# DataIntensive-HPC/abft-sparse-cg

Measured on AMD Instinct MI355X. Metric: CG iterations/sec + SpMV effective HBM GB/s (% of roofline), 1/2/4/8 MI355X, higher is better.
Workload: dtype f64; 1 GPU; cg-csr -t hip -m none, synthetic laplace5:3162,3162; N=9998244, nnz=49978572, format=csr, mode=none, parallelism=1 GPU

## Files before the change

### abft_sparse_cg_amd/capi.py

```python
import ctypes as C
import os

_HERE = os.path.dirname(os.path.abspath(__file__))
LIB_PATH = os.environ.get("ABFT_HIP_LIB") or os.path.join(_HERE, "libabft_hip.so")
HEADER_PATH = os.path.join(os.path.dirname(_HERE), "include", "abft_hip.h")

OK = 0
MODES = ("none", "constraints", "sed", "sec7", "sec8", "secded")
MODE_ID = {m: i for i, m in enumerate(MODES)}
MODE_ID["sec"] = MODE_ID["sec7"]
FMT_CSR, FMT_COO = 0, 1
FLIP_ANY, FLIP_VALUE, FLIP_INDEX = 0, 1, 2
PART_ALL, PART_INTERIOR, PART_BOUNDARY = 0, 1, 2
K_SPMV, K_DOT, K_CALC_XR, K_CALC_P = 0, 1, 2, 3
EV_VEC_CORRECTED, EV_VEC_DOUBLE = 10, 11
FMT_VECTOR = 2
MAX_RHS = 8

u32p = C.POINTER(C.c_uint32)
f64p = C.POINTER(C.c_double)
i32p = C.POINTER(C.c_int)
vp = C.c_void_p
vpp = C.POINTER(C.c_void_p)

# ... 78 lines not shown
    "abft_hip_calc_px_precond_block": (C.c_int, [vp, vp, vp, vp, vp, C.c_int, f64p, f64p, C.c_uint32]),
    "abft_hip_dot_dev": (C.c_int, [vp, vp, vp, vp]),
    "abft_hip_calc_xr_dev": (C.c_int, [vp, vp, vp, vp, vp, C.c_double, vp]),
    "abft_hip_read_pair": (C.c_int, [vp, vp, f64p, f64p]),
    "abft_hip_spmv_dot_dev": (C.c_int, [vp, vp, vp, vp, C.c_int, vp]),
    "abft_hip_matrix_set_interior": (C.c_int, [vp, C.c_int, C.c_int]),
    "abft_hip_spmv_part": (C.c_int, [vp, vp, vp, vp, C.c_int]),
    "abft_hip_spmv_dot_part_dev": (C.c_int, [vp, vp, vp, vp, C.c_int, vp, C.c_int]),
    "abft_hip_calc_xr_ratio_dev": (C.c_int, [vp, vp, vp, vp, vp, vp, vp, vp]),
    "abft_hip_calc_p_ratio_dev": (C.c_int, [vp, vp, vp, vp, vp]),
    "abft_hip_set_sharers": (C.c_int, [vp, C.c_int]),
    "abft_hip_speculation_stats": (C.c_int, [vp, C.POINTER(C.c_long), C.POINTER(C.c_long)]),
    "abft_hip_cg_iteration_dev": (C.c_int, [vp, vp, vp, C.c_int, C.c_int, vp, vp, vp, vp, vp, vp, vp]),
    "abft_hip_tail_stats": (C.c_int, [vp, i32p, i32p, i32p, C.POINTER(C.c_long)]),
    "abft_hip_x_in_spmv_stats": (C.c_int, [vp, C.POINTER(C.c_long), C.POINTER(C.c_long)]),
    "abft_hip_cg_iteration_until_dev": (C.c_int, [vp, vp, vp, C.c_int, C.c_int, vp, vp, vp, vp, vp, vp, vp, C.c_double]),
    "abft_hip_write_pair": (C.c_int, [vp, vp, C.c_double, C.c_double]),
    "abft_hip_peer_board_bytes": (C.c_size_t, []),
    "abft_hip_peer_board_attach": (C.c_int, [vp, vp, C.c_size_t, C.c_int, C.c_int, C.c_double]),
    "abft_hip_peer_board_detach": (C.c_int, [vp]),
    "abft_hip_allreduce_pair_peers": (C.c_int, [vp, vp]),
    "abft_hip_peer_board_failed": (C.c_int, [vp]),
    "abft_hip_peer_board_ipc_handle_bytes": (C.c_size_t, []),
    "abft_hip_peer_board_ipc_export": (C.c_int, [vp, vp]),
    "abft_hip_peer_board_ipc_attach": (C.c_int, [vp, vp, C.c_int, C.c_int, C.c_double]),
    "abft_hip_peer_board_device_alloc": (C.c_int, [vp, C.POINTER(vp)]),
    "abft_hip_peer_board_device_free": (C.c_int, [vp, vp]),
    "abft_hip_peer_board_attach_device": (C.c_int, [vp, C.POINTER(vp), C.c_int, C.c_int, C.c_double]),
    "abft_hip_peer_board_fuse": (C.c_int, [vp, C.c_int]),
    "abft_hip_peer_exchange_bytes": (C.c_size_t, [C.c_int, C.c_size_t]),
# ... 81 lines not shown
```

### abft_sparse_cg_amd/context.py

```python
import ctypes as C
import math
import sys

import numpy as np

from . import capi
from .capi import FMT_COO, FMT_CSR, MODE_ID, check


class FatalEvent(SystemExit):

    def __init__(self, events):
        super().__init__(1)
        self.events = events


class ResidualCheckFailed(RuntimeError):

    def __init__(self, message, checks):
        super().__init__(message)
        self.checks = checks


class Matrix:
# ... 424 lines not shown
    def stream_probe(self, nbytes=1 << 30, reps=10):
        c, r = C.c_double(), C.c_double()
        check(self.L.abft_hip_stream_probe(self.h, nbytes, reps, C.byref(c), C.byref(r)))
        return c.value, r.value

    def tail_stats(self):
        path, grid, want = C.c_int(0), C.c_int(0), C.c_int(0)
        counts = (C.c_long * 4)()
        check(self.L.abft_hip_tail_stats(self.h, C.byref(path), C.byref(grid), C.byref(want), counts))
        return path.value, grid.value, want.value, list(counts)

    def x_in_spmv_stats(self):
        absorbed, flushed = C.c_long(0), C.c_long(0)
        check(self.L.abft_hip_x_in_spmv_stats(self.h, C.byref(absorbed), C.byref(flushed)))
        return absorbed.value, flushed.value

    def cg_iteration_until_dev(self, mat, vec, x, r, p, w, scalars, rr_at, pw_at, rr_new_at, threshold, vec_offset=0,
                               part=capi.PART_ALL):
        base = scalars.device_ptr
        check(self.L.abft_hip_cg_iteration_until_dev(self.h, mat.h, vec.h, vec_offset, part, x.h, r.h, p.h, w.h,
                                                     base + 8 * rr_at, base + 8 * pw_at, base + 8 * rr_new_at,
                                                     threshold))

    def graph_begin(self):
        check(self.L.abft_hip_graph_begin(self.h))

    def graph_end(self):
        g = C.c_void_p()
        check(self.L.abft_hip_graph_end(self.h, C.byref(g)))
        return g
# ... 368 lines not shown
```

### abft_sparse_cg_amd/csrc/abft_hip.hip

```cpp
#include <algorithm>
#include <array>
#include <chrono>
#include <cmath>
#include <cstdarg>
#include <cstdio>
#include <cstdlib>
#include <cstring>
#include <new>
#include <thread>
#include <map>
#include <mutex>
#include <vector>

#include "abft_internal.h"


static thread_local char g_err[512] = "";

static int set_err(int code, const char *fmt, ...) {
  va_list ap;
  va_start(ap, fmt);
  vsnprintf(g_err, sizeof(g_err), fmt, ap);
  va_end(ap);
  return code;
// ... 36 lines not shown
  HostSlot *host_slot_dev = nullptr;
  struct {
    bool enabled = false;
    bool learned = false;
    abft_hip_vector *x = nullptr, *r = nullptr, *p = nullptr, *w = nullptr;
    bool have_rr = false;
    int rr_at = 0;
    double rr_host = 0.0;
    int stage = 0;
    uint32_t seq_rr = 0;
    double rr_new_host = 0.0;
    double *shadow[2] = {nullptr, nullptr};
    int shadow_n = 0;
    double *scal = nullptr;
    long commits = 0, drops = 0;
  } spec;
  EventRing ring{};
  MovedList moved{};
  int *bits_dev = nullptr;
  bool fuse_enabled = true;
  struct {
    bool valid = false, have_value = false;
    bool vecc = false;
    const double *x = nullptr, *y = nullptr;
    int n = 0;
    uint32_t seq = 0;
    double value = 0.0;
  } fused;
  bool defer_enabled = true;
  struct {
// ... 115 lines not shown
  return ABFT_OK;
}

static int flush_deferred(abft_hip_ctx *ctx) {
  if (!ctx->defer.active) return ABFT_OK;
  ctx->defer.active = false;
  HIPCHK(launch_axpy(ctx->defer.x, ctx->defer.p, ctx->defer.alpha, ctx->defer.on_dev ? ctx->alpha_dev : nullptr,
                     ctx->defer.n, ctx->stream));
  return ABFT_OK;
}

static bool same_bits(double a, double b) { return memcmp(&a, &b, sizeof(a)) == 0; }

static void spec_drop(abft_hip_ctx *ctx) {
  auto &S = ctx->spec;
  if (S.stage) S.drops++;
  if (S.stage == 2) {
    S.rr_at = 1 - S.rr_at;
    S.rr_host = S.rr_new_host;
  }
  S.stage = 0;
}
static void spec_forget(abft_hip_ctx *ctx) {
  spec_drop(ctx);
  ctx->spec.learned = false;
  ctx->spec.have_rr = false;
  ctx->spec.x = ctx->spec.r = ctx->spec.p = ctx->spec.w = nullptr;
}

static int bind(abft_hip_ctx *ctx, bool keep_deferred = false, bool keep_spec = false, bool keep_xpend = false) {
  if (!ctx) return set_err(ABFT_ERR_INVALID, "null context");
  HIPCHK(hipSetDevice(ctx->device));
  ctx->xpend.prev_p = ctx->xpend.last_p;
  ctx->xpend.last_p = nullptr;
  if (!keep_spec) spec_drop(ctx);
  if (!keep_deferred && !keep_xpend)
    if (int rc = flush_xpend(ctx)) return rc;
  if (!keep_deferred) return flush_deferred(ctx);
  return ABFT_OK;
}
// ... 120 lines not shown
  if (const char *e = getenv("ABFT_HIP_TAIL")) ctx->tail_enabled = strcmp(e, "0") != 0;
  if (const char *e = getenv("ABFT_HIP_SYNC")) ctx->spin_wait = strcmp(e, "stream") != 0;
  if (const char *e = getenv("ABFT_HIP_FUSE_DOT")) ctx->fuse_enabled = strcmp(e, "0") != 0;
  if (const char *e = getenv("ABFT_HIP_FUSE_X")) ctx->defer_enabled = strcmp(e, "0") != 0;
  HIPCHK(hipMalloc((void **)&ctx->alpha_dev, sizeof(double)));
  HIPCHK(hipHostMalloc((void **)&ctx->host_slot, ABFT_HOST_SLOTS * sizeof(HostSlot), hipHostMallocMapped | hipHostMallocCoherent));
  memset(ctx->host_slot, 0, ABFT_HOST_SLOTS * sizeof(HostSlot));
  HIPCHK(hipMalloc((void **)&ctx->spec.scal, 8 * sizeof(double)));
  HIPCHK(hipMemset(ctx->spec.scal, 0, 8 * sizeof(double)));
  if (const char *e = getenv("ABFT_HIP_SPECULATE")) ctx->spec.enabled = strcmp(e, "0") != 0;
  if (const char *e = getenv("ABFT_HIP_X_IN_SPMV")) {
    ctx->xin_enabled = strcmp(e, "0") != 0;
    if (ctx->xin_enabled) ctx->xin_modes = ~0u;
  }
  ctx->xin_enabled = ctx->xin_enabled && ctx->defer_enabled && ctx->fuse_enabled && !ctx->spec.enabled;
  HIPCHK(hipHostGetDevicePointer((void **)&ctx->host_slot_dev, ctx->host_slot, 0));
  HIPCHK(hipMalloc((void **)&ctx->ring.buf, EVENT_CAP * sizeof(abft_event) + VECC_SEEN_BYTES));
  HIPCHK(hipMalloc((void **)&ctx->ring.count, sizeof(uint32_t)));
  HIPCHK(hipMemset(ctx->ring.count, 0, sizeof(uint32_t)));
  HIPCHK(hipMemset(ctx->ring.buf + EVENT_CAP, 0, VECC_SEEN_BYTES));
  ctx->ring.cap = EVENT_CAP;
  HIPCHK(hipMalloc((void **)&ctx->moved.buf, 2 * (size_t)MOVED_CAP * sizeof(MovedEntry)));
  HIPCHK(hipMalloc((void **)&ctx->moved.count, sizeof(uint32_t)));
  HIPCHK(hipMemset(ctx->moved.count, 0, sizeof(uint32_t)));
  ctx->moved.cap = MOVED_CAP;
  HIPCHK(hipMalloc((void **)&ctx->bits_dev, 32 * sizeof(int)));
  {
    double *scratch = nullptr;
    HIPCHK(hipMalloc((void **)&scratch, 8 * sizeof(double)));
    HIPCHK(hipMemset(scratch, 0, 8 * sizeof(double)));
// ... 1414 lines not shown
                     disjoint(x, p) && disjoint(x, w) && disjoint(r, p);
  KernelTimer t(ctx, ABFT_K_CALC_XR);
  if (defer) {
    HIPCHK(launch_calc_r(r->d, w->d, alpha, num, den, num ? ctx->alpha_dev : nullptr, x->n, o, ctx->stream, nullptr, x->d, p->d));
    ctx->defer.active = true;
    ctx->defer.on_dev = num != nullptr;
    ctx->defer.x = x->d; ctx->defer.p = p->d; ctx->defer.n = x->n; ctx->defer.alpha = alpha;
    return ABFT_OK;
  }
  HIPCHK(launch_calc_xr(x->d, r->d, p->d, w->d, alpha, num, den, x->n, o, ctx->stream));
  return ABFT_OK;
}

static bool spec_plain(const abft_hip_vector *v, int n);

static bool xpend_take(abft_hip_ctx *ctx, abft_hip_vector *p, const abft_hip_vector *r, double beta, int *rc) {
  auto &X = ctx->xpend;
  *rc = ABFT_OK;
  if (!ctx->xin_enabled || !X.armed || X.active || ctx->defer.on_dev || ctx->capturing) return false;
  if (!spec_plain(p, p->n) || !disjoint(p, r)) return false;
  int at = X.shadow[0].buf && X.shadow[0].n == p->n ? 0 : X.shadow[1].buf && X.shadow[1].n == p->n ? 1 : -1;
  if (at < 0) {
    at = X.shadow[X.shadow_at].buf ? 1 - X.shadow_at : X.shadow_at;
    (void)hipFree(X.shadow[at].buf);
    X.shadow[at].buf = nullptr;
    X.shadow[at].n = 0;
    if (hipMalloc((void **)&X.shadow[at].buf, ((size_t)p->n + 2) * sizeof(double)) != hipSuccess) {
      (void)hipGetLastError();
      X.shadow[at].buf = nullptr;
      ctx->xin_enabled = false;
      return false;
    }
    X.shadow[at].n = p->n;
  }
  X.shadow_at = at;
  {
    KernelTimer t(ctx, ABFT_K_CALC_P);
    const hipError_t e = launch_calc_p(p->d, r->d, beta, nullptr, nullptr, p->n, ctx->stream, X.shadow[at].buf);
    if (e != hipSuccess) {
      *rc = set_err(ABFT_ERR_HIP, "calc_p: %s", hipGetErrorString(e));
      return true;
    }
  }
  std::swap(p->d, X.shadow[at].buf);
  X.active = true;
  X.x = ctx->defer.x; X.p_old = X.shadow[at].buf; X.alpha = ctx->defer.alpha; X.n = p->n; X.ph = p;
  return true;
}

static int calc_p_launch(abft_hip_ctx *ctx, abft_hip_vector *p, const abft_hip_vector *r, double beta,
// ... 13 lines not shown
        ctx->xpend.last_p = p;
        if (taken) return ABFT_OK;
      }
      KernelTimer t(ctx, ABFT_K_CALC_P);
      HIPCHK(launch_calc_px(p->d, r->d, ctx->defer.x, beta, num, den, ctx->defer.alpha,
                            ctx->defer.on_dev ? ctx->alpha_dev : nullptr, p->n, ctx->stream));
      return ABFT_OK;
    }
    if (int rc = flush_deferred(ctx)) return rc;
  }
  KernelTimer t(ctx, ABFT_K_CALC_P);
  HIPCHK(launch_calc_p(p->d, r->d, beta, num, den, p->n, ctx->stream));
  return ABFT_OK;
}

extern "C" int abft_hip_calc_xr(abft_hip_ctx *ctx, abft_hip_vector *x, abft_hip_vector *r, const abft_hip_vector *p,
                                const abft_hip_vector *w, double alpha, double *result) {
  if (int rc = bind(ctx, false, true)) return rc;
  if (!result) { spec_drop(ctx); return set_err(ABFT_ERR_INVALID, "null result"); }
  auto &S = ctx->spec;
  if (S.stage == 1) {
    bool take = x == S.x && r == S.r && p == S.p && w == S.w && ctx->fused.valid;
    if (take && !ctx->fused.have_value) {
      take = scalar_from_host_slot(ctx, ctx->fused.seq, &ctx->fused.value) == ABFT_OK;
      ctx->fused.have_value = take;
    }
    take = take && same_bits(alpha, S.rr_host / ctx->fused.value);
    if (take) {
      {
        double *rr = S.scal + 2 * S.rr_at, *rr_dev_new = S.scal + 2 * (1 - S.rr_at);
        KernelTimer t(ctx, ABFT_K_CALC_P);
        HIPCHK(launch_calc_px(p->d, S.shadow[0], x->d, 0.0, rr_dev_new, rr, 0.0, ctx->alpha_dev, x->n, ctx->stream, S.shadow[1],
                              nullptr));
      }
      double rr_new = 0.0;
      if (int rc = scalar_from_host_slot(ctx, S.seq_rr, &rr_new)) { spec_drop(ctx); return rc; }
      std::swap(r->d, S.shadow[0]);
      ctx->fused.valid = false;
      S.stage = 2;
      S.rr_new_host = rr_new;
      *result = rr_new;
      return ABFT_OK;
    }
    spec_drop(ctx);
  } else
    spec_drop(ctx);
  const int at = S.have_rr ? 1 - S.rr_at : 0;
  const ReduceOut o = reduce_out(ctx, S.scal + 2 * at, true);
  if (int rc = calc_xr_launch(ctx, x, r, p, w, alpha, o)) { S.have_rr = false; return rc; }
  if (int rc = scalar_from_host_slot(ctx, o.seq, result)) { S.have_rr = false; return rc; }
  S.have_rr = true; S.rr_at = at; S.rr_host = *result;
  S.x = x; S.r = r; S.p = const_cast<abft_hip_vector *>(p); S.w = const_cast<abft_hip_vector *>(w);
  S.learned = false;
  return ABFT_OK;
}

extern "C" int abft_hip_calc_xr_dev(abft_hip_ctx *ctx, abft_hip_vector *x, abft_hip_vector *r,
                                    const abft_hip_vector *p, const abft_hip_vector *w, double alpha,
                                    double *dev_result) {
  if (int rc = bind(ctx)) return rc;
  if (!dev_result) return set_err(ABFT_ERR_INVALID, "null result");
  return calc_xr_launch(ctx, x, r, p, w, alpha, reduce_out(ctx, dev_result, false));
}

extern "C" int abft_hip_calc_p(abft_hip_ctx *ctx, abft_hip_vector *p, const abft_hip_vector *r, double beta) {
  if (int rc = bind(ctx, true, true)) return rc;
  auto &S = ctx->spec;
  if (S.stage == 2) {
    const bool take = p == S.p && r == S.r && same_bits(beta, S.rr_new_host / S.rr_host) && !ctx->defer.active;
    if (take) {
      std::swap(p->d, S.shadow[1]);
      ctx->fused.valid = false;
      S.stage = 0;
      S.rr_at = 1 - S.rr_at;
      S.rr_host = S.rr_new_host;
      S.commits++;
      return ABFT_OK;
    }
    spec_drop(ctx);
  } else
    spec_drop(ctx);
  const bool completes = S.have_rr && !S.learned && S.p == p && S.r == r && S.x && S.w;
  if (int rc = calc_p_launch(ctx, p, r, beta, nullptr, nullptr)) return rc;
  S.learned = completes || (S.learned && S.p == p && S.r == r);
  return ABFT_OK;
}

extern "C" int abft_hip_read_pair(abft_hip_ctx *ctx, const double *dev_pair, double *value, double *events) {
  if (int rc = bind(ctx, true)) return rc;
  if (!dev_pair || !value) return set_err(ABFT_ERR_INVALID, "null argument");
  if (!ctx->fused.have_value) ctx->fused.valid = false;
  const uint32_t seq = ++ctx->seq;
  HIPCHK(launch_publish_pair(dev_pair, ctx->host_slot_dev + (seq % ABFT_HOST_SLOTS), seq, ctx->stream));
  if (int rc = scalar_from_host_slot(ctx, seq, value)) return rc;
  if (events) *events = (double)ctx->host_slot[seq % ABFT_HOST_SLOTS].evcount;
  return ABFT_OK;
}

// ... 514 lines not shown
  }
  S.stage = 1;
  S.seq_rr = o.seq;
  return ABFT_OK;
}

struct HeldFold {
  bool held = false;
  FuseOut fuse{};
  uint32_t nparts = 0;
  FixArgs fix{};
};

static bool xpend_predicted(abft_hip_ctx *ctx, const abft_hip_matrix *mat, const abft_hip_vector *vec,
                            const abft_hip_vector *result, const double *dev_pair, int part, int c1, bool held,
                            bool vecc) {
  auto &X = ctx->xpend;
  const abft_hip_vector *after_calc_p = X.prev_p;
  X.prev_p = nullptr;
  if (!ctx->xin_enabled || !mat || !vec || !result) return false;
  if (mat->fmt != ABFT_FMT_CSR || mat->use_slice || mat->use_sweep || mat->use_panels) return false;
  if (!(ctx->xin_modes >> (unsigned)mat->mode & 1u)) return false;
  if (part != ABFT_PART_ALL || c1 >= 0 || dev_pair || held || vecc || ctx->capturing) return false;
  const uint32_t n = mat->csr.n_out;
  if (!mat->fuse_partials || !ctx->fuse_enabled || n == 0 || mat->csr.n_in != n || mat->csr.nblk == 0 ||
      (uint32_t)vec->n != n || (uint32_t)result->n != n || !disjoint(vec, result))
    return false;
  if (!X.active) {
    if (after_calc_p == vec && spec_plain(vec, vec->n)) X.armed = true;
    return false;
  }
  abft_hip_vector xv, pv;
  xv.d = X.x; xv.n = X.n;
  pv.d = const_cast<double *>(X.p_old); pv.n = X.n;
  return X.ph == vec && (uint32_t)X.n == n && disjoint(&xv, result) && disjoint(&pv, result);
}

static int spmv_common(abft_hip_ctx *ctx, abft_hip_matrix *mat, const abft_hip_vector *vec,
                       abft_hip_vector *result, int vec_offset, double *dev_pair, int part = ABFT_PART_ALL,
                       int c0 = 0, int c1 = -1, HeldFold *hold = nullptr, bool vecc = false) {
  if (int rc = bind(ctx, false, false, true)) return rc;
  const bool absorb = xpend_predicted(ctx, mat, vec, result, dev_pair, part, c1, hold != nullptr, vecc);
  if (!absorb)
    if (int rc = flush_xpend(ctx)) return rc;
  if (!mat || !vec || !result) return set_err(ABFT_ERR_INVALID, "spmv: null argument");
  if (vecc) {
    spec_forget(ctx);
    const char *layout = mat->fmt != ABFT_FMT_CSR ? "COO" : mat->use_slice ? "slice" : mat->use_sweep ? "sweep"
                         : mat->use_panels ? "panel" : nullptr;
    if (layout)
      return set_err(ABFT_ERR_INVALID, "spmv_vecc: a matrix in the %s layout (protected vectors run on CSR matrices "
                     "in the streaming layout only)", layout);
    if (!disjoint(vec, result)) return set_err(ABFT_ERR_INVALID, "spmv_vecc: input and output overlap");
  }
  if (part < ABFT_PART_ALL || part > ABFT_PART_BOUNDARY) return set_err(ABFT_ERR_INVALID, "spmv: unknown part %d", part);
  const uint32_t n_out = mat->fmt == ABFT_FMT_CSR ? mat->csr.n_out : mat->coo.n_out;
  const uint32_t n_in = mat->fmt == ABFT_FMT_CSR ? mat->csr.n_in : mat->coo.n_in;
// ... 88 lines not shown
    KernelTimer t(ctx, ABFT_K_DOT);
    ReduceOut big{};
    big.partials = ctx->partials; big.ticket = ctx->ticket; big.dev_out = fuse.dev_out; big.host = fuse.host;
    big.ev_count = fuse.ev_count; big.seq = fuse.seq; big.peers = fuse.peers;
    HIPCHK(launch_fuse_finalize(fuse, nparts, big, fix.on ? &fix : nullptr, ctx->stream));
  }
  if (to_host && do_fuse) {
    ctx->fused.valid = true;
    ctx->fused.have_value = false;
    ctx->fused.vecc = vecc;
    ctx->fused.x = vec->d;
    ctx->fused.y = result->d;
    ctx->fused.n = vec->n;
    ctx->fused.seq = fuse.seq;
    if (whole && part == ABFT_PART_ALL && !vecc) (void)spec_launch(ctx, vec, result);
  }
  return ABFT_OK;
}

extern "C" int abft_hip_spmv(abft_hip_ctx *ctx, abft_hip_matrix *mat, const abft_hip_vector *vec,
                             abft_hip_vector *result) {
  return spmv_common(ctx, mat, vec, result, 0, nullptr);
}

extern "C" int abft_hip_spmv_dot_dev(abft_hip_ctx *ctx, abft_hip_matrix *mat, const abft_hip_vector *vec,
                                     abft_hip_vector *result, int vec_offset, double *dev_result) {
  if (!dev_result) return set_err(ABFT_ERR_INVALID, "null result");
  return spmv_common(ctx, mat, vec, result, vec_offset, dev_result);
}

// ... 862 lines not shown
    ReduceOut big{};
    big.partials = ctx->partials; big.ticket = ctx->ticket; big.dev_out = hold.fuse.dev_out; big.host = hold.fuse.host;
    big.ev_count = hold.fuse.ev_count; big.seq = hold.fuse.seq; big.peers = hold.fuse.peers;
    HIPCHK(launch_fuse_finalize(hold.fuse, hold.nparts, big, hold.fix.on ? &hold.fix : nullptr, ctx->stream));
  }
  const ReduceOut o = reduce_out(ctx, dev_rr_new, false);
  {
    KernelTimer t(ctx, ABFT_K_CALC_XR);
    HIPCHK(launch_calc_r_until(r->d, w->d, dev_rr, dev_pw, threshold, ctx->alpha_dev, n, o, ctx->stream, x->d, p->d));
  }
  KernelTimer t(ctx, ABFT_K_CALC_P);
  HIPCHK(launch_calc_px_until(p->d, r->d, x->d, dev_rr, dev_rr_new, threshold, ctx->alpha_dev, n, ctx->stream));
  return ABFT_OK;
}

extern "C" int abft_hip_x_in_spmv_stats(abft_hip_ctx *ctx, long *absorbed, long *flushed) {
  if (!ctx) return set_err(ABFT_ERR_INVALID, "null context");
  if (absorbed) *absorbed = ctx->xpend.absorbed;
  if (flushed) *flushed = ctx->xpend.flushed;
  return ABFT_OK;
}


struct abft_hip_graph {
  abft_hip_ctx *ctx = nullptr;
  hipGraph_t graph = nullptr;
  hipGraphExec_t exec = nullptr;
};

extern "C" int abft_hip_graph_begin(abft_hip_ctx *ctx) {
// ... 230 lines not shown
```

### abft_sparse_cg_amd/csrc/abft_internal.h

```cpp
#pragma once
#include <hip/hip_runtime.h>
#include <stdint.h>

#include "../../include/abft_hip.h"

struct EventRing {
  abft_event *buf;
  uint32_t *count;
  uint32_t cap;
};

#define ABFT_VECC_SEEN_SLOTS 4096u
#define ABFT_VECC_SEEN_PROBES 8u

struct CsrDev {
  uint32_t *cols;
  double *vals;
  const uint32_t *rowptr;
  const uint4 *blk;
  uint32_t nblk, n_out, n_in, nnz, index_base;
  const uint32_t *orig_index;
  const uint32_t *pos_of_orig;
  const uint32_t *gidx;
};
// ... 100 lines not shown
#endif
#ifndef ABFT_CFG_SWEEP_COUNTS_NT
#define ABFT_CFG_SWEEP_COUNTS_NT 0
#endif
#ifndef ABFT_CFG_PX_OUT_NT
#define ABFT_CFG_PX_OUT_NT 0
#endif
#ifndef ABFT_X_IN_SPMV_MODES
#define ABFT_X_IN_SPMV_MODES 0x01u
#endif
#ifndef ABFT_CFG_XUPD_NT
#define ABFT_CFG_XUPD_NT 7
#endif
#ifndef ABFT_CFG_P_OUT_NT
#define ABFT_CFG_P_OUT_NT 1
#endif
#ifndef ABFT_CFG_X_NT
#define ABFT_CFG_X_NT 0
#endif
#ifndef ABFT_CFG_COO_LEAN_WAVES
#define ABFT_CFG_COO_LEAN_WAVES 8
#endif
#ifndef ABFT_CFG_COO_PANEL_XPF_AHEAD
#define ABFT_CFG_COO_PANEL_XPF_AHEAD 1
#endif
#ifndef ABFT_CFG_COO_PANEL_PREFETCH
#define ABFT_CFG_COO_PANEL_PREFETCH 0
#endif
#ifndef ABFT_CFG_COO_SCHED_BARRIER
#define ABFT_CFG_COO_SCHED_BARRIER 1
// ... 276 lines not shown
```

### abft_sparse_cg_amd/csrc/kernels.hip

```cpp
#include <type_traits>

#include "abft_internal.h"
#include "ecc_device.h"

typedef double f64x2 __attribute__((ext_vector_type(2)));
typedef uint32_t u32x2 __attribute__((ext_vector_type(2)));
typedef uint32_t u32x4 __attribute__((ext_vector_type(4)));

#if ABFT_CFG_NT
#define STREAM_LOAD(p) __builtin_nontemporal_load(p)
#else
#define STREAM_LOAD(p) (*(p))
#endif

#ifndef ABFT_CFG_GATHER
#define ABFT_CFG_GATHER 0
#endif
__device__ __forceinline__ double gather_load(const double *p) {
#if ABFT_CFG_GATHER == 1
  return __builtin_nontemporal_load(p);
#elif ABFT_CFG_GATHER == 2
  return __hip_atomic_load(p, __ATOMIC_RELAXED, __HIP_MEMORY_SCOPE_AGENT);
#else
  return *p;
// ... 690 lines not shown
        if (re > A.nnz) { push_event(ev, ABFT_EV_ROW_SIZE, row, row, FMT_CSR); continue; }
        if (re < rs) { push_event(ev, ABFT_EV_ROW_ORDER, row, row, FMT_CSR); continue; }
      }
      if (rs < e0 || re > e1 || re < rs) continue;
      double acc = 0.0;
      if (csr_row_sum<MODE>(A, ev, base, rs, re, re, s_prod, s_col, acc, row)) {
        if (VECC) {
          const uint64_t yw = vecc_encode(acc);
          y[row] = vecc_double(yw);
          if (FUSE) {
            uint64_t xw = vecc_bits(xr);
            if (__builtin_expect(vecc_suspect(xw) != 0u, 0)) xw = vecc_cold(xw, fuse.x_off + row, 0u, ev).w;
            dsum += vecc_value(xw) * vecc_value(yw);
          }
        } else {
          y[row] = acc;
          if (FUSE) dsum += xr * acc;
        }
      }
    }
  } else {
    if (XUPD)
      for (uint32_t row = row0 + threadIdx.x; row < row1; row += ABFT_BLOCK) XUPD_STORE_X(xu.xs + row, XUPD_LOAD_X(xu.xs + row) + xu.alpha * XUPD_LOAD_P(xu.p_old + row));
    for (uint32_t row = row0; row < row1; row++) {
      const uint32_t rs = A.rowptr[row], re = A.rowptr[row + 1];
      if (MODE == MODE_CONSTRAINTS) {
        if (re > A.nnz) { if (threadIdx.x == 0) push_event(ev, ABFT_EV_ROW_SIZE, row, row, FMT_CSR); continue; }
        if (re < rs) { if (threadIdx.x == 0) push_event(ev, ABFT_EV_ROW_ORDER, row, row, FMT_CSR); continue; }
      }
      if (re > A.nnz || re < rs) continue;
      double acc = 0.0;
// ... 2326 lines not shown
  if (num) alpha = *num / *den;
  if (alpha_out && blockIdx.x == 0 && threadIdx.x == 0) *alpha_out = alpha;
  double acc = 0.0;
  const long stride = (long)gridDim.x * ABFT_BLOCK * VEC;
  for (long i = ((long)blockIdx.x * ABFT_BLOCK + threadIdx.x) * VEC; i < n; i += stride) {
    if (VEC == 2 && i + 1 < n) {
      double2 rv = *reinterpret_cast<const double2 *>(r + i);
#if ABFT_CFG_DEAD_NT & 1
      typedef double v2d __attribute__((ext_vector_type(2)));
      const v2d wl = __builtin_nontemporal_load(reinterpret_cast<const v2d *>(w + i));
      const double2 wv = make_double2(wl.x, wl.y);
#else
      const double2 wv = *reinterpret_cast<const double2 *>(w + i);
#endif
      rv.x -= alpha * wv.x; rv.y -= alpha * wv.y;
      *reinterpret_cast<double2 *>(r_out + i) = rv;
      acc += rv.x * rv.x;
      acc += rv.y * rv.y;
    } else {
      const double rs = r[i] - alpha * w[i];
      r_out[i] = rs;
      acc += rs * rs;
    }
  }
  acc = block_sum(acc, s_w);
  reduce_finish(acc, out, s_w);
}

template <int VEC>
__global__ __launch_bounds__(ABFT_BLOCK) void calc_px_kernel(const double *p, const double *__restrict__ r,
                                                             const double *x, double beta,
// ... 1921 lines not shown
```

### include/abft_hip.h

```cpp
#ifndef ABFT_HIP_H
#define ABFT_HIP_H

#include <stddef.h>
#include <stdint.h>

#ifdef __cplusplus
extern "C" {
#endif

#define ABFT_OK 0
#define ABFT_ERR_INVALID (-1)
#define ABFT_ERR_HIP (-2)
#define ABFT_ERR_NOMEM (-3)
#define ABFT_ERR_RANGE (-4)
#define ABFT_ERR_NODEVICE (-5)

typedef enum {
  ABFT_MODE_NONE = 0,
  ABFT_MODE_CONSTRAINTS = 1,
  ABFT_MODE_SED = 2,
  ABFT_MODE_SEC7 = 3,
  ABFT_MODE_SEC8 = 4,
  ABFT_MODE_SECDED = 5
} abft_mode;
// ... 233 lines not shown
int abft_hip_matrix_panels(abft_hip_matrix *mat, int *npanels, int *width);
int abft_hip_spmv_dot_range_dev(abft_hip_ctx *ctx, abft_hip_matrix *mat, const abft_hip_vector *vec,
                                abft_hip_vector *result, int vec_offset, double *dev_result, int c0, int c1);

int abft_hip_speculation_stats(abft_hip_ctx *ctx, long *taken, long *dropped);

int abft_hip_set_sharers(abft_hip_ctx *ctx, int processes);

int abft_hip_cg_iteration_dev(abft_hip_ctx *ctx, abft_hip_matrix *mat, const abft_hip_vector *vec, int vec_offset,
                              int part, abft_hip_vector *x, abft_hip_vector *r, abft_hip_vector *p,
                              abft_hip_vector *w, const double *dev_rr, double *dev_pw, double *dev_rr_new);
int abft_hip_tail_stats(abft_hip_ctx *ctx, int *path, int *grid, int *want, long counts[4]);

int abft_hip_x_in_spmv_stats(abft_hip_ctx *ctx, long *absorbed, long *flushed);

int abft_hip_cg_iteration_until_dev(abft_hip_ctx *ctx, abft_hip_matrix *mat, const abft_hip_vector *vec,
                                    int vec_offset, int part, abft_hip_vector *x, abft_hip_vector *r,
                                    abft_hip_vector *p, abft_hip_vector *w, const double *dev_rr,
                                    double *dev_pw, double *dev_rr_new, double threshold);


typedef struct abft_hip_graph abft_hip_graph;
int abft_hip_graph_begin(abft_hip_ctx *ctx);
int abft_hip_graph_end(abft_hip_ctx *ctx, abft_hip_graph **graph);
int abft_hip_graph_launch(abft_hip_graph *graph);
int abft_hip_graph_destroy(abft_hip_graph *graph);


int abft_hip_drain_events(abft_hip_ctx *ctx, abft_event *buf, int cap, int *count, int *fatal);
int abft_hip_event_capacity(void);
// ... 26 lines not shown
```

### profiles/summarize.py

```python
#!/usr/bin/env python3
import csv
import glob
import json
import os
import re
import sys
from collections import defaultdict


def short(name):
    name = re.sub(r"\(.*", "", name)
    name = name.replace("void ", "").replace(" [clone .kd]", "").replace(".kd", "")
    return name.strip()


def find(d, pattern):
    return sorted(glob.glob(os.path.join(d, "**", pattern), recursive=True))


def trace(d, out):
    rows = defaultdict(list)
    for f in find(d, "*kernel_trace.csv"):
        for r in csv.DictReader(open(f)):
            rows[short(r["Kernel_Name"])].append(int(r["End_Timestamp"]) - int(r["Start_Timestamp"]))
    tot = sum(sum(v) for v in rows.values()) or 1
    with open(out, "w") as o:
        o.write("| kernel | launches | total ms | avg us | min us | max us | % |\n|---|---|---|---|---|---|---|\n")
        for k, v in sorted(rows.items(), key=lambda kv: -sum(kv[1])):
            o.write("| `%s` | %d | %.3f | %.2f | %.2f | %.2f | %.1f |\n" % (
                k, len(v), sum(v) / 1e6, sum(v) / len(v) / 1e3, min(v) / 1e3, max(v) / 1e3, 100.0 * sum(v) / tot))
    print(open(out).read())


def pmc(d, out):
    acc = defaultdict(lambda: defaultdict(list))
    for f in find(d, "*counter_collection.csv"):
        for r in csv.DictReader(open(f)):
            acc[short(r["Kernel_Name"])][r["Counter_Name"]].append(float(r["Counter_Value"]))
    res = {k: {c: {"avg_per_launch": sum(v) / len(v), "launches": len(v)} for c, v in cs.items()}
           for k, cs in acc.items()}
    json.dump(res, open(out, "w"), indent=1, sort_keys=True)
    for k, cs in res.items():
        for c, v in cs.items():
            print("%-60s %-18s %14.1f  (%d launches)" % (k[:60], c, v["avg_per_launch"], v["launches"]))

# ... 12 lines not shown
    for n, disp in enumerate(sorted(per)):
        for c, v in per[disp].items():
            acc[n % k][c].append(v)
    res = {"phase %d" % ph: {c: {"avg_per_launch": sum(v) / len(v), "launches": len(v)} for c, v in cs.items()}
           for ph, cs in acc.items()}
    json.dump(res, open(out, "w"), indent=1, sort_keys=True)
    for ph in sorted(res):
        for c, v in res[ph].items():
            print("%-10s %-18s %14.1f  (%d launches)" % (ph, c, v["avg_per_launch"], v["launches"]))


if __name__ == "__main__":
    if sys.argv[1] == "pmc_phases":
        pmc_phases(*sys.argv[2:6])
    else:
        {"trace": trace, "pmc": pmc}[sys.argv[1]](sys.argv[2], sys.argv[3])
```

Baseline: 4834 CG iterations/s.

## Speculatively launch next direction update ahead of host scalar readback

Adds an 'ahead' speculation path. After calc_xr it enqueues calc_p into a shadow buffer, with beta computed on the device from the new and old residual norms, and commits it by pointer swap when the host later calls calc_p with a matching beta. An optional level 2 also runs the residual update right after SpMV, using alpha computed on the device. The aim is to remove the idle gaps where the GPU waits for the host to read the scalars and launch the next kernel. It adds bookkeeping and drop paths, and wasted work on mispredictions. Optional nontemporal store switches for r and y and a profiling gap analyzer are also added, but are off or outside the measured path by default.

```diff
diff --git a/abft_sparse_cg_amd/capi.py b/abft_sparse_cg_amd/capi.py
--- a/abft_sparse_cg_amd/capi.py
+++ b/abft_sparse_cg_amd/capi.py
@@ -116,6 +116,7 @@
     "abft_hip_cg_iteration_dev": (C.c_int, [vp, vp, vp, C.c_int, C.c_int, vp, vp, vp, vp, vp, vp, vp]),
     "abft_hip_tail_stats": (C.c_int, [vp, i32p, i32p, i32p, C.POINTER(C.c_long)]),
     "abft_hip_x_in_spmv_stats": (C.c_int, [vp, C.POINTER(C.c_long), C.POINTER(C.c_long)]),
+    "abft_hip_ahead_stats": (C.c_int, [vp, C.POINTER(C.c_long), C.POINTER(C.c_long), C.POINTER(C.c_long)]),
     "abft_hip_cg_iteration_until_dev": (C.c_int, [vp, vp, vp, C.c_int, C.c_int, vp, vp, vp, vp, vp, vp, vp, C.c_double]),
     "abft_hip_write_pair": (C.c_int, [vp, vp, C.c_double, C.c_double]),
     "abft_hip_peer_board_bytes": (C.c_size_t, []),
diff --git a/abft_sparse_cg_amd/context.py b/abft_sparse_cg_amd/context.py
--- a/abft_sparse_cg_amd/context.py
+++ b/abft_sparse_cg_amd/context.py
@@ -462,6 +462,11 @@
         absorbed, flushed = C.c_long(0), C.c_long(0)
         check(self.L.abft_hip_x_in_spmv_stats(self.h, C.byref(absorbed), C.byref(flushed)))
         return absorbed.value, flushed.value
+
+    def ahead_stats(self):
+        cp, cr, d = C.c_long(0), C.c_long(0), C.c_long(0)
+        check(self.L.abft_hip_ahead_stats(self.h, C.byref(cp), C.byref(cr), C.byref(d)))
+        return cp.value, cr.value, d.value
 
     def cg_iteration_until_dev(self, mat, vec, x, r, p, w, scalars, rr_at, pw_at, rr_new_at, threshold, vec_offset=0,
                                part=capi.PART_ALL):
diff --git a/abft_sparse_cg_amd/csrc/abft_hip.hip b/abft_sparse_cg_amd/csrc/abft_hip.hip
--- a/abft_sparse_cg_amd/csrc/abft_hip.hip
+++ b/abft_sparse_cg_amd/csrc/abft_hip.hip
@@ -74,6 +74,12 @@
     int shadow_n = 0;
     double *scal = nullptr;
     long commits = 0, drops = 0;
+    int ahead = ABFT_AHEAD_DEFAULT;
+    bool a_armed = false;
+    bool a_alpha_ok = false;
+    double rr_prev = 0.0;
+    int a_slot = 0;
+    long a_commit_p = 0, a_commit_r = 0, a_drops = 0;
   } spec;
   EventRing ring{};
   MovedList moved{};
@@ -219,6 +225,13 @@
 
 static void spec_drop(abft_hip_ctx *ctx) {
   auto &S = ctx->spec;
+  S.a_alpha_ok = false;
+  if (S.stage >= 3) {
+    S.a_drops++;
+    S.a_armed = false;
+    S.stage = 0;
+    return;
+  }
   if (S.stage) S.drops++;
   if (S.stage == 2) {
     S.rr_at = 1 - S.rr_at;
@@ -229,6 +242,7 @@
 static void spec_forget(abft_hip_ctx *ctx) {
   spec_drop(ctx);
   ctx->spec.learned = false;
+  ctx->spec.a_armed = false;
   ctx->spec.have_rr = false;
   ctx->spec.x = ctx->spec.r = ctx->spec.p = ctx->spec.w = nullptr;
 }
@@ -379,6 +393,8 @@
     if (ctx->xin_enabled) ctx->xin_modes = ~0u;
   }
   ctx->xin_enabled = ctx->xin_enabled && ctx->defer_enabled && ctx->fuse_enabled && !ctx->spec.enabled;
+  if (const char *e = getenv("ABFT_HIP_AHEAD")) ctx->spec.ahead = e[0] == '2' ? 2 : e[0] == '1' ? 1 : 0;
+  if (!ctx->xin_enabled) ctx->spec.ahead = 0;
   HIPCHK(hipHostGetDevicePointer((void **)&ctx->host_slot_dev, ctx->host_slot, 0));
   HIPCHK(hipMalloc((void **)&ctx->ring.buf, EVENT_CAP * sizeof(abft_event) + VECC_SEEN_BYTES));
   HIPCHK(hipMalloc((void **)&ctx->ring.count, sizeof(uint32_t)));
@@ -1823,26 +1839,33 @@
 
 static bool spec_plain(const abft_hip_vector *v, int n);
 
+static int xpend_buffer(abft_hip_ctx *ctx, int n) {
+  auto &X = ctx->xpend;
+  int at = X.shadow[0].buf && X.shadow[0].n == n ? 0 : X.shadow[1].buf && X.shadow[1].n == n ? 1 : -1;
+  if (at < 0) {
+    at = X.shadow[X.shadow_at].buf ? 1 - X.shadow_at : X.shadow_at;
+    (void)hipFree(X.shadow[at].buf);
+    X.shadow[at].buf = nullptr;
+    X.shadow[at].n = 0;
+    if (hipMalloc((void **)&X.shadow[at].buf, ((size_t)n + 2) * sizeof(double)) != hipSuccess) {
+      (void)hipGetLastError();
+      X.shadow[at].buf = nullptr;
+      ctx->xin_enabled = false;
+      return -1;
+    }
+    X.shadow[at].n = n;
+  }
+  X.shadow_at = at;
+  return at;
+}
+
 static bool xpend_take(abft_hip_ctx *ctx, abft_hip_vector *p, const abft_hip_vector *r, double beta, int *rc) {
   auto &X = ctx->xpend;
   *rc = ABFT_OK;
   if (!ctx->xin_enabled || !X.armed || X.active || ctx->defer.on_dev || ctx->capturing) return false;
   if (!spec_plain(p, p->n) || !disjoint(p, r)) return false;
-  int at = X.shadow[0].buf && X.shadow[0].n == p->n ? 0 : X.shadow[1].buf && X.shadow[1].n == p->n ? 1 : -1;
-  if (at < 0) {
-    at = X.shadow[X.shadow_at].buf ? 1 - X.shadow_at : X.shadow_at;
-    (void)hipFree(X.shadow[at].buf);
-    X.shadow[at].buf = nullptr;
-    X.shadow[at].n = 0;
-    if (hipMalloc((void **)&X.shadow[at].buf, ((size_t)p->n + 2) * sizeof(double)) != hipSuccess) {
-      (void)hipGetLastError();
-      X.shadow[at].buf = nullptr;
-      ctx->xin_enabled = false;
-      return false;
-    }
-    X.shadow[at].n = p->n;
-  }
-  X.shadow_at = at;
+  const int at = xpend_buffer(ctx, p->n);
+  if (at < 0) return false;
   {
     KernelTimer t(ctx, ABFT_K_CALC_P);
     const hipError_t e = launch_calc_p(p->d, r->d, beta, nullptr, nullptr, p->n, ctx->stream, X.shadow[at].buf);
@@ -1886,12 +1909,86 @@
   return ABFT_OK;
 }
 
+static bool ahead_plain(const abft_hip_vector *x, const abft_hip_vector *r, const abft_hip_vector *p,
+                        const abft_hip_vector *w) {
+  if (!p || p->n <= 0) return false;
+  const int n = p->n;
+  return spec_plain(x, n) && spec_plain(r, n) && spec_plain(p, n) && spec_plain(w, n) && x != r && x != p && x != w &&
+         r != p && r != w && p != w;
+}
+
+static bool ahead_p_launch(abft_hip_ctx *ctx, const abft_hip_vector *p, const double *r_d, const double *num,
+                           const double *den) {
+  auto &X = ctx->xpend;
+  if (!ctx->xin_enabled || !X.armed || X.active || ctx->capturing) return false;
+  const int at = xpend_buffer(ctx, p->n);
+  if (at < 0) return false;
+  KernelTimer t(ctx, ABFT_K_CALC_P);
+  if (launch_calc_p(p->d, r_d, 0.0, num, den, p->n, ctx->stream, X.shadow[at].buf) != hipSuccess) return false;
+  ctx->spec.a_slot = at;
+  return true;
+}
+
+static void ahead_launch(abft_hip_ctx *ctx, const abft_hip_vector *vec, const abft_hip_vector *result) {
+  auto &S = ctx->spec;
+  if (S.ahead < 2 || !S.a_armed || S.stage || !S.have_rr || ctx->defer.active || ctx->capturing) return;
+  if (vec != S.p || result != S.w || !ahead_plain(S.x, S.r, S.p, S.w)) return;
+  if (!ctx->xin_enabled || !ctx->xpend.armed || ctx->xpend.active) return;
+  const int n = vec->n;
+  if (S.shadow_n != n || !S.shadow[0]) {
+    (void)hipFree(S.shadow[0]);
+    S.shadow[0] = nullptr;
+    S.shadow_n = 0;
+    if (hipMalloc((void **)&S.shadow[0], ((size_t)n + 2) * sizeof(double)) != hipSuccess) {
+      (void)hipGetLastError();
+      S.shadow[0] = nullptr;
+      S.ahead = 1;
+      return;
+    }
+    S.shadow_n = n;
+  }
+  if (xpend_buffer(ctx, n) < 0) return;
+  double *rr = S.scal + 2 * S.rr_at, *rr_new = S.scal + 2 * (1 - S.rr_at), *pw = S.scal + 4;
+  const ReduceOut o = reduce_out(ctx, rr_new, true);
+  {
+    KernelTimer t(ctx, ABFT_K_CALC_XR);
+    if (launch_calc_r(S.r->d, S.w->d, 0.0, rr, pw, nullptr, n, o, ctx->stream, S.shadow[0], S.x->d, S.p->d) != hipSuccess) return;
+  }
+  S.seq_rr = o.seq;
+  S.stage = 4;
+  if (!ahead_p_launch(ctx, S.p, S.shadow[0], rr_new, rr)) spec_drop(ctx);
+}
+
 extern "C" int abft_hip_calc_xr(abft_hip_ctx *ctx, abft_hip_vector *x, abft_hip_vector *r, const abft_hip_vector *p,
                                 const abft_hip_vector *w, double alpha, double *result) {
   if (int rc = bind(ctx, false, true)) return rc;
   if (!result) { spec_drop(ctx); return set_err(ABFT_ERR_INVALID, "null result"); }
   auto &S = ctx->spec;
-  if (S.stage == 1) {
+  const bool had_rr = S.have_rr;
+  const double rr_old = S.rr_host;
+  const bool alpha_ok = S.ahead && had_rr && ctx->fused.valid && ctx->fused.have_value && !ctx->fused.vecc && p && w &&
+                        ctx->fused.x == p->d && ctx->fused.y == w->d && alpha == alpha &&
+                        same_bits(alpha, rr_old / ctx->fused.value) && ahead_plain(x, r, p, w);
+  if (S.stage == 4) {
+    if (alpha_ok && x == S.x && r == S.r && p == S.p && w == S.w) {
+      double rr_new = 0.0;
+      if (int rc = scalar_from_host_slot(ctx, S.seq_rr, &rr_new)) { spec_drop(ctx); return rc; }
+      std::swap(r->d, S.shadow[0]);
+      ctx->fused.valid = false;
+      ctx->defer.active = true;
+      ctx->defer.on_dev = false;
+      ctx->defer.x = x->d; ctx->defer.p = p->d; ctx->defer.n = x->n; ctx->defer.alpha = alpha;
+      S.rr_prev = rr_old;
+      S.rr_at = 1 - S.rr_at;
+      S.rr_host = rr_new;
+      S.stage = 3;
+      S.a_alpha_ok = true;
+      S.a_commit_r++;
+      *result = rr_new;
+      return ABFT_OK;
+    }
+    spec_drop(ctx);
+  } else if (S.stage == 1) {
     bool take = x == S.x && r == S.r && p == S.p && w == S.w && ctx->fused.valid;
     if (take && !ctx->fused.have_value) {
       take = scalar_from_host_slot(ctx, ctx->fused.seq, &ctx->fused.value) == ABFT_OK;
@@ -1920,7 +2017,13 @@
   const int at = S.have_rr ? 1 - S.rr_at : 0;
   const ReduceOut o = reduce_out(ctx, S.scal + 2 * at, true);
   if (int rc = calc_xr_launch(ctx, x, r, p, w, alpha, o)) { S.have_rr = false; return rc; }
+  if (!alpha_ok) S.a_armed = false;
+  const bool p_ahead = alpha_ok && S.a_armed && ctx->defer.active && !ctx->defer.on_dev && ctx->defer.p == p->d &&
+                       ahead_p_launch(ctx, p, r->d, S.scal + 2 * at, S.scal + 2 * S.rr_at);
   if (int rc = scalar_from_host_slot(ctx, o.seq, result)) { S.have_rr = false; return rc; }
+  if (p_ahead) S.stage = 3;
+  S.a_alpha_ok = alpha_ok;
+  S.rr_prev = rr_old;
   S.have_rr = true; S.rr_at = at; S.rr_host = *result;
   S.x = x; S.r = r; S.p = const_cast<abft_hip_vector *>(p); S.w = const_cast<abft_hip_vector *>(w);
   S.learned = false;
@@ -1938,7 +2041,24 @@
 extern "C" int abft_hip_calc_p(abft_hip_ctx *ctx, abft_hip_vector *p, const abft_hip_vector *r, double beta) {
   if (int rc = bind(ctx, true, true)) return rc;
   auto &S = ctx->spec;
-  if (S.stage == 2) {
+  const bool beta_ok = S.a_alpha_ok && p == S.p && r == S.r && beta == beta && same_bits(beta, S.rr_host / S.rr_prev) &&
+                       ahead_plain(S.x, S.r, S.p, S.w);
+  if (S.stage == 3) {
+    auto &X = ctx->xpend;
+    if (beta_ok && ctx->defer.active && !ctx->defer.on_dev && ctx->defer.p == p->d && ctx->defer.n == p->n && !X.active) {
+      const int at = S.a_slot;
+      ctx->defer.active = false;
+      std::swap(p->d, X.shadow[at].buf);
+      X.active = true;
+      X.x = ctx->defer.x; X.p_old = X.shadow[at].buf; X.alpha = ctx->defer.alpha; X.n = p->n; X.ph = p;
+      X.last_p = p;
+      ctx->fused.valid = false;
+      S.stage = 0;
+      S.a_commit_p++;
+      return ABFT_OK;
+    }
+    spec_drop(ctx);
+  } else if (S.stage == 2) {
     const bool take = p == S.p && r == S.r && same_bits(beta, S.rr_new_host / S.rr_host) && !ctx->defer.active;
     if (take) {
       std::swap(p->d, S.shadow[1]);
@@ -1954,6 +2074,7 @@
     spec_drop(ctx);
   const bool completes = S.have_rr && !S.learned && S.p == p && S.r == r && S.x && S.w;
   if (int rc = calc_p_launch(ctx, p, r, beta, nullptr, nullptr)) return rc;
+  S.a_armed = S.ahead && beta_ok;
   S.learned = completes || (S.learned && S.p == p && S.r == r);
   return ABFT_OK;
 }
@@ -2498,7 +2619,7 @@
 
 static bool xpend_predicted(abft_hip_ctx *ctx, const abft_hip_matrix *mat, const abft_hip_vector *vec,
                             const abft_hip_vector *result, const double *dev_pair, int part, int c1, bool held,
-                            bool vecc) {
+                            bool vecc, bool *eligible) {
   auto &X = ctx->xpend;
   const abft_hip_vector *after_calc_p = X.prev_p;
   X.prev_p = nullptr;
@@ -2510,6 +2631,7 @@
   if (!mat->fuse_partials || !ctx->fuse_enabled || n == 0 || mat->csr.n_in != n || mat->csr.nblk == 0 ||
       (uint32_t)vec->n != n || (uint32_t)result->n != n || !disjoint(vec, result))
     return false;
+  *eligible = true;
   if (!X.active) {
     if (after_calc_p == vec && spec_plain(vec, vec->n)) X.armed = true;
     return false;
@@ -2524,7 +2646,8 @@
                        abft_hip_vector *result, int vec_offset, double *dev_pair, int part = ABFT_PART_ALL,
                        int c0 = 0, int c1 = -1, HeldFold *hold = nullptr, bool vecc = false) {
   if (int rc = bind(ctx, false, false, true)) return rc;
-  const bool absorb = xpend_predicted(ctx, mat, vec, result, dev_pair, part, c1, hold != nullptr, vecc);
+  bool absorb_ok = false;
+  const bool absorb = xpend_predicted(ctx, mat, vec, result, dev_pair, part, c1, hold != nullptr, vecc, &absorb_ok);
   if (!absorb)
     if (int rc = flush_xpend(ctx)) return rc;
   if (!mat || !vec || !result) return set_err(ABFT_ERR_INVALID, "spmv: null argument");
@@ -2643,6 +2766,7 @@
     ctx->fused.n = vec->n;
     ctx->fused.seq = fuse.seq;
     if (whole && part == ABFT_PART_ALL && !vecc) (void)spec_launch(ctx, vec, result);
+    if (absorb_ok) ahead_launch(ctx, vec, result);
   }
   return ABFT_OK;
 }
@@ -3535,6 +3659,14 @@
   return ABFT_OK;
 }
 
+extern "C" int abft_hip_ahead_stats(abft_hip_ctx *ctx, long *committed_p, long *committed_r, long *dropped) {
+  if (!ctx) return set_err(ABFT_ERR_INVALID, "null context");
+  if (committed_p) *committed_p = ctx->spec.a_commit_p;
+  if (committed_r) *committed_r = ctx->spec.a_commit_r;
+  if (dropped) *dropped = ctx->spec.a_drops;
+  return ABFT_OK;
+}
+
 extern "C" int abft_hip_x_in_spmv_stats(abft_hip_ctx *ctx, long *absorbed, long *flushed) {
   if (!ctx) return set_err(ABFT_ERR_INVALID, "null context");
   if (absorbed) *absorbed = ctx->xpend.absorbed;
diff --git a/abft_sparse_cg_amd/csrc/abft_internal.h b/abft_sparse_cg_amd/csrc/abft_internal.h
--- a/abft_sparse_cg_amd/csrc/abft_internal.h
+++ b/abft_sparse_cg_amd/csrc/abft_internal.h
@@ -138,6 +138,15 @@
 #endif
 #ifndef ABFT_CFG_P_OUT_NT
 #define ABFT_CFG_P_OUT_NT 1
+#endif
+#ifndef ABFT_CFG_R_NT
+#define ABFT_CFG_R_NT 0
+#endif
+#ifndef ABFT_CFG_Y_NT
+#define ABFT_CFG_Y_NT 0
+#endif
+#ifndef ABFT_AHEAD_DEFAULT
+#define ABFT_AHEAD_DEFAULT 1
 #endif
 #ifndef ABFT_CFG_X_NT
 #define ABFT_CFG_X_NT 0
diff --git a/abft_sparse_cg_amd/csrc/kernels.hip b/abft_sparse_cg_amd/csrc/kernels.hip
--- a/abft_sparse_cg_amd/csrc/kernels.hip
+++ b/abft_sparse_cg_amd/csrc/kernels.hip
@@ -728,7 +728,8 @@
             dsum += vecc_value(xw) * vecc_value(yw);
           }
         } else {
-          y[row] = acc;
+          if (ABFT_CFG_Y_NT && XUPD && MODE == MODE_NONE) __builtin_nontemporal_store(acc, y + row);
+          else y[row] = acc;
           if (FUSE) dsum += xr * acc;
         }
       }
@@ -3085,7 +3086,14 @@
       const double2 wv = *reinterpret_cast<const double2 *>(w + i);
 #endif
       rv.x -= alpha * wv.x; rv.y -= alpha * wv.y;
+#if ABFT_CFG_R_NT
+      typedef double v2r __attribute__((ext_vector_type(2)));
+      if ((ABFT_CFG_R_NT & 1) && r_out != r) __builtin_nontemporal_store(v2r{rv.x, rv.y}, reinterpret_cast<v2r *>(r_out + i));
+      else if ((ABFT_CFG_R_NT & 2) && r_out == r) __builtin_nontemporal_store(v2r{rv.x, rv.y}, reinterpret_cast<v2r *>(r_out + i));
+      else *reinterpret_cast<double2 *>(r_out + i) = rv;
+#else
       *reinterpret_cast<double2 *>(r_out + i) = rv;
+#endif
       acc += rv.x * rv.x;
       acc += rv.y * rv.y;
     } else {
diff --git a/include/abft_hip.h b/include/abft_hip.h
--- a/include/abft_hip.h
+++ b/include/abft_hip.h
@@ -271,6 +271,8 @@
 
 int abft_hip_x_in_spmv_stats(abft_hip_ctx *ctx, long *absorbed, long *flushed);
 
+int abft_hip_ahead_stats(abft_hip_ctx *ctx, long *committed_p, long *committed_r, long *dropped);
+
 int abft_hip_cg_iteration_until_dev(abft_hip_ctx *ctx, abft_hip_matrix *mat, const abft_hip_vector *vec,
                                     int vec_offset, int part, abft_hip_vector *x, abft_hip_vector *r,
                                     abft_hip_vector *p, abft_hip_vector *w, const double *dev_rr,
diff --git a/profiles/summarize.py b/profiles/summarize.py
--- a/profiles/summarize.py
+++ b/profiles/summarize.py
@@ -29,6 +29,28 @@
         for k, v in sorted(rows.items(), key=lambda kv: -sum(kv[1])):
             o.write("| `%s` | %d | %.3f | %.2f | %.2f | %.2f | %.1f |\n" % (
                 k, len(v), sum(v) / 1e6, sum(v) / len(v) / 1e3, min(v) / 1e3, max(v) / 1e3, 100.0 * sum(v) / tot))
+    print(open(out).read())
+
+
+def gaps(d, out, min_share=0.02):
+    rows = []
+    for f in find(d, "*kernel_trace.csv"):
+        for r in csv.DictReader(open(f)):
+            rows.append((int(r["Start_Timestamp"]), int(r["End_Timestamp"]), short(r["Kernel_Name"])))
+    rows.sort()
+    pairs = defaultdict(list)
+    for (s0, e0, k0), (s1, e1, k1) in zip(rows, rows[1:]):
+        pairs[(k0, k1)].append(s1 - e0)
+    keep = {k: sorted(v) for k, v in pairs.items() if len(v) >= min_share * len(rows)}
+    per_iter = max((len(v) for v in keep.values()), default=1)
+    with open(out, "w") as o:
+        o.write("| kernel | next kernel | pairs | mean gap us | median us | us per iteration |\n|---|---|---|---|---|---|\n")
+        total = 0.0
+        for (k0, k1), v in sorted(keep.items(), key=lambda kv: -sum(kv[1])):
+            total += sum(v) / per_iter / 1e3
+            o.write("| `%s` | `%s` | %d | %.2f | %.2f | %.2f |\n" % (
+                k0, k1, len(v), sum(v) / len(v) / 1e3, v[len(v) // 2] / 1e3, sum(v) / per_iter / 1e3))
+        o.write("\nidle between kernels: %.2f us per iteration (%d iterations)\n" % (total, per_iter))
     print(open(out).read())
 
 
@@ -71,4 +93,4 @@
     if sys.argv[1] == "pmc_phases":
         pmc_phases(*sys.argv[2:6])
     else:
-        {"trace": trace, "pmc": pmc}[sys.argv[1]](sys.argv[2], sys.argv[3])
+        {"trace": trace, "pmc": pmc, "gaps": gaps}[sys.argv[1]](sys.argv[2], sys.argv[3])
```

Result: faster. 4976 CG iterations/s, median of 6 (+2.9%).
